# AVianEco/Softspoken

Measured on AMD Instinct MI355X. Metric: audio-seconds processed/sec (whole node), 16 kHz mono, higher is better.
Workload: dtype f16x2

## Files before the change

softspoken_amd/csrc/conv4.hip:

```cpp
#include "conv4_forms.h"
#include <cstdio>
#include <cstdlib>
#include <type_traits>
#include <utility>

namespace ss {

static constexpr int kMfmaPrio = 2;
__device__ __forceinline__ uint32_t relu_pk(uint32_t v) {
    return __builtin_bit_cast(uint32_t, __builtin_elementwise_max(__builtin_bit_cast(s16x2, v), s16x2{0, 0}));
}
__device__ __forceinline__ uint32_t max_pk(uint32_t a, uint32_t b) {
    return __builtin_bit_cast(uint32_t, __builtin_elementwise_max(__builtin_bit_cast(s16x2, a), __builtin_bit_cast(s16x2, b)));
}

template <int NT, int NW, bool BRES, bool RES, bool RADD, bool POOL, int RP, bool FIRST, bool FLAT, bool PF2, bool SPLIT = false, bool RANK1 = false,
          int NH = 1, bool GRES = false>
__global__ __launch_bounds__(64 * NW * NH) __attribute__((amdgpu_waves_per_eu((NT <= 2 && !(SPLIT && RES && !BRES && NW == 4 && NH == 1)) ? 4 : 2)))
void conv3x3_v4_kernel(ConvArgs a, int total_tiles, int lds_b_bytes) {
    constexpr int KC = 32;
    constexpr bool DUO = NH > 1;
    static_assert(!DUO || (NT == 1 && NW * NH == 16 && (RP == 0 || (GRES && RP == 1 && POOL)) && !FIRST && !FLAT && !PF2),
                  "DUO: the plain A / B launches; GRES also conv2_1.B's projection in B");
    static_assert(!GRES || (DUO && BRES && SPLIT && !RES), "GRES: f16x2 B launches with resident banks");
    constexpr bool RING = DUO && !BRES;
    static_assert(!RING || (SPLIT && NH == 4), "RING: f16x2, four 4-wave tiles");
    static_assert(!SPLIT || !PF2, "SPLIT: single-stage prefetch");
    static_assert(!RANK1 || (SPLIT && !RES && !RADD), "RANK1: conv1_1.B in f16x2 mode");
    static_assert(!(FIRST && SPLIT) || RANK1, "FIRST in f16x2 mode: the block's residual is the fp32 rank-1 term");
    static_assert(!FLAT || (NT == 1 && NW == 8 && BRES && (RADD || RP) && !POOL && !FIRST), "FLAT: conv9_1.B");
    static_assert(!PF2 || (BRES && !FIRST), "two-stage prefetch: resident-weight launches");
    static_assert(RP == 0 || (!RES && !RADD && !FIRST), "RP: a B launch that computes the block's projection itself (no r tensor)");
    static_assert(!FIRST || (NT == 1 && BRES && !RES && !RADD), "FIRST: conv1_1.B, one 32 -> 32 chunk, rank-1 residual");
    constexpr int kTapBytes = 2 * NT * 1024;
    constexpr int TAPS = RES ? 10 : 9;
    constexpr int NTHR = 64 * NW;
    constexpr int TH = 2 * NW;
    constexpr int PR = TH + 2;
    constexpr int kA = PR * kRowPitch;
    constexpr int NPA = PR * kPatch * 4;
    constexpr int AIT = (NPA + NTHR - 1) / NTHR;
    constexpr int NPB = (SPLIT ? 2 : 1) * TAPS * kTapBytes / 16;
    constexpr int BIT = BRES ? 1 : (DUO ? (NPB / 2 + NTHR - 1) / NTHR : (NPB + NTHR - 1) / NTHR);
    static_assert(!(RES && (RADD || POOL)), "RES is the A launch; RADD / POOL belong to B launches");
    static_assert(AIT <= 4, "edge flags are packed 8 bits per piece");
    extern __shared__ __attribute__((aligned(16))) char smem[];

    const int half = DUO ? __builtin_amdgcn_readfirstlane((int)threadIdx.x / NTHR) : 0;
    const int tid = DUO ? (int)threadIdx.x % NTHR : (int)threadIdx.x, lane = tid & 63;
    const int wave = __builtin_amdgcn_readfirstlane(tid >> 6);
    const int hh = lane >> 5, m = lane & 31;
    const int py = (m >> 1) & 1, px = (m & 1) | ((m >> 2) << 1);
    char* sA = smem + half * kA;
    const int sb_bytes = RING ? 2 * lds_b_bytes : lds_b_bytes;
    char* sB = smem + NH * kA;
    const int proj_steps = RP ? (a.C0x + a.C1x) / 16 : 0;
    constexpr bool proj_lds = RP > 0 && (BRES || NT == 3 || SPLIT);
    const char* sProj = smem + NH * kA + sb_bytes;
    const int proj_tiles = SPLIT ? a.Cout / 32 : NT;
    const int proj_bank = proj_steps * proj_tiles * 1024;
    const float* sBias = (const float*)(sProj + (proj_lds ? (SPLIT ? 2 : 1) * proj_bank : 0));
    constexpr int FW = 20, FROWS = PR + 3;
    float* sFb = (float*)sBias + 32;
    float* sF = sFb + 32;
    float* sFlat = (float*)sBias + 32;

    const int H = a.H, W = a.W, Cout = a.Cout;
    const int ngroups = Cout / (32 * NT);
    const int nch_r = (a.C0 + a.C1) / KC;
    const int nch = SPLIT ? 2 * nch_r : nch_r;
    const int all_taps = nch_r * TAPS;

    const int xcd = blockIdx.x & 7, local = (int)(blockIdx.x >> 3) * NH + half, gper = (int)(gridDim.x >> 3) * NH;
    const int per = (total_tiles + 7) >> 3;
#ifdef SS_DEVBUILD
// ... 424 lines not shown
                const int tiles = Cout / 32;
#pragma unroll
                for (int k = 0; k < RP; ++k) {
                    const int sidx = ci * RP + k < proj_steps ? ci * RP + k : 0;
#pragma unroll
                    for (int nt = 0; nt < NT; ++nt)
                        wpg[k][nt] = *(const u32x4*)((const char*)a.proj_w + ((size_t)(sidx * tiles + cur.g * NT + nt) * 64 + lane) * 16);
                }
            }
        }
        if (ci == 0) {
#pragma unroll
            for (int nt = 0; nt < NT; ++nt)
#pragma unroll
                for (int g = 0; g < 4; ++g) {
                    const f32x4 b4 = *(const f32x4*)(sBias + co0 + nt * 32 + 8 * g + 4 * hh);
                    acc[nt][4 * g] = b4[0]; acc[nt][4 * g + 1] = b4[1]; acc[nt][4 * g + 2] = b4[2]; acc[nt][4 * g + 3] = b4[3];
                    if constexpr (RES) {
                        const f32x4 r4 = *(const f32x4*)(sBias + Cout + co0 + nt * 32 + 8 * g + 4 * hh);
                        racc[nt][4 * g] = r4[0]; racc[nt][4 * g + 1] = r4[1]; racc[nt][4 * g + 2] = r4[2]; racc[nt][4 * g + 3] = r4[3];
                    }
                }
        }
        auto proj_products = [&](auto k0c, auto k1c) {
            constexpr int K0 = decltype(k0c)::value, K1 = decltype(k1c)::value;
#pragma unroll
            for (int k = K0; k < K1; ++k) {
                const int sidx = (ci >> 1) * RP + k < proj_steps ? (ci >> 1) * RP + k : 0;
#pragma unroll
                for (int nt = 0; nt < NT; ++nt) {
                    const int wt = (sidx * proj_tiles + (int)(co0 >> 5) + nt) * 1024 + lane * 16;
                    const u32x4 wh = *(const u32x4*)(sProj + wt), wl = *(const u32x4*)(sProj + proj_bank + wt);
                    acc[nt] = mfma16<true>(wh, pxl[k - K0], acc[nt]);
                    acc[nt] = mfma16<true>(wl, pxh[k - K0], acc[nt]);
                    acc[nt] = mfma16<true>(wh, pxh[k - K0], acc[nt]);
                }
            }
        };
        using KZ_ = std::integral_constant<int, 0>; using KH_ = std::integral_constant<int, RPH>; using KR_ = std::integral_constant<int, RP>;
        if constexpr (SPLIT && RP > 0 && PART == 1) {
            proj_products(KZ_{}, KH_{});
            __builtin_amdgcn_sched_barrier(0);
            if constexpr (RP > RPH) issue_proj(cur, ci >> 1, KH_{}, KR_{});
        }
        if constexpr (FLAT && SPLIT && RP > 0) load_flat_w();
        {
            const char* bbase = sB + boff0 + (BRES ? ((DUO && !GRES ? cur.g * nch : 0) + (SPLIT ? (ci >> 1) * 2 : ci)) * TAPS * kTapBytes
                                                   : RING ? ((stage_no >> 1) & 1) * lds_b_bytes : 0);
            constexpr int PD = (NT == 1) ? 4 : 2;
            u32x4 af[PD], bfr[PD][NT];
            u32x4 rfr[RES ? 2 : 1][RES ? NT : 1];
            if (a.dbg & 32) __builtin_amdgcn_s_setprio(kMfmaPrio);
            constexpr bool kMerged = SPLIT && NSTEP == 36 && NT == 1;
            if constexpr (kMerged) {
                constexpr int PM = 3;
                u32x4 pf[PM], wh_[PM], wl_[PM], rh_[RES ? 2 : 1], rl_[RES ? 2 : 1];
                const char* bb0 = bbase; const char* bb1 = bbase + TAPS * kTapBytes;
                auto load3 = [&](int st, int slot) {
                    const int tap = st >> 1, sub = st & 1, dy = tap / 3, dx = tap % 3;
                    pf[slot] = *(const u32x4*)(sA + aoff0 + dy * kRowPitch + dx * kPixPitch + sub * 32);
                    wh_[slot] = *(const u32x4*)(bb0 + tap * kTapBytes + sub * 1024);
                    wl_[slot] = *(const u32x4*)(bb1 + tap * kTapBytes + sub * 1024);
                };
#pragma unroll
                for (int st = 0; st < PM - 1; ++st) load3(st, st);
#pragma unroll
                for (int st = 0; st < 18; ++st) {
                    if (st + PM - 1 < 18) load3(st + PM - 1, (st + PM - 1) % PM);
                    if constexpr (RES) {
                        if (st == 6) {
#pragma unroll
                            for (int sub = 0; sub < 2; ++sub) {
                                rh_[sub] = *(const u32x4*)(bb0 + 9 * kTapBytes + sub * 1024);
                                rl_[sub] = *(const u32x4*)(bb1 + 9 * kTapBytes + sub * 1024);
                            }
                        }
                    }
                    const u32x4 pixv = pf[st % PM];
                    acc[0] = mfma16<true>(wh_[st % PM], pixv, acc[0]);
                    acc[0] = mfma16<true>(wl_[st % PM], pixv, acc[0]);
                    if constexpr (RES) {
                        if (st == 8 || st == 9) {
                            racc[0] = mfma16<true>(rh_[st & 1], pixv, racc[0]);
                            racc[0] = mfma16<true>(rl_[st & 1], pixv, racc[0]);
                        }
                    }
                }
            } else
#pragma unroll
            for (int bank = 0; bank < NSTEP / 18; ++bank) {
                const char* bb = bbase + bank * TAPS * kTapBytes;
                auto load_frags = [&](int st, u32x4& fa, u32x4 (&fbb)[NT]) {
                    const int tap = st >> 1, sub = st & 1, dy = tap / 3, dx = tap % 3;
                    fa = *(const u32x4*)(sA + aoff0 + dy * kRowPitch + dx * kPixPitch + sub * 32);
#pragma unroll
                    for (int nt = 0; nt < NT; ++nt) fbb[nt] = *(const u32x4*)(bb + tap * kTapBytes + (sub * NT + nt) * 1024);
                };
                if (bank) __builtin_amdgcn_sched_barrier(0);
#pragma unroll
                for (int st = 0; st < PD - 1; ++st) load_frags(st, af[st], bfr[st]);
#pragma unroll
                for (int st = 0; st < 18; ++st) {
                    if (st + PD - 1 < 18) load_frags(st + PD - 1, af[(st + PD - 1) % PD], bfr[(st + PD - 1) % PD]);
                    if constexpr (RES) {
                        if (st == 6) {
#pragma unroll
                            for (int sub = 0; sub < 2; ++sub)
#pragma unroll
                                for (int nt = 0; nt < NT; ++nt) rfr[sub][nt] = *(const u32x4*)(bb + 9 * kTapBytes + (sub * NT + nt) * 1024);
                        }
                    }
                    const u32x4 pixv = af[st % PD];
#pragma unroll
                    for (int nt = 0; nt < NT; ++nt) {
                        acc[nt] = mfma16<SPLIT>(bfr[st % PD][nt], pixv, acc[nt]);
                        if constexpr (RES) {
                            if (st == 8 || st == 9) racc[nt] = mfma16<SPLIT>(rfr[st & 1][nt], pixv, racc[nt]);
                        }
                    }
                }
            }
        }

        if constexpr (SPLIT && RP > RPH && PART == 1) proj_products(KH_{}, KR_{});
        if constexpr (RP > 0 && !SPLIT) {
#pragma unroll
            for (int k = 0; k < RP; ++k) {
                const int sidx = ci * RP + k < proj_steps ? ci * RP + k : 0;
#pragma unroll
                for (int nt = 0; nt < NT; ++nt) {
                    u32x4 wp;
                    if constexpr (proj_lds) wp = *(const u32x4*)(sProj + (sidx * NT + nt) * 1024 + lane * 16); else wp = wpg[k][nt];
                    acc[nt] = __builtin_amdgcn_mfma_f32_32x32x16_bf16(__builtin_bit_cast(bf16x8, wp), __builtin_bit_cast(bf16x8, xf[k]), acc[nt], 0, 0, 0);
                }
            }
        }
        if (a.dbg & 32) __builtin_amdgcn_s_setprio(0);
        if constexpr (FIRST && !SPLIT) {
            const float f = sF[(2 * wave + py + 2) * FW + px + 2];
// ... 294 lines not shown
            return false;
        }
        cs = n1; n1 = n2; ok1 = ok2;
        if constexpr (PF2) { n2 = n3; ok2 = ok3; }
        return true;
    };
    using P0 = std::integral_constant<int, 0>; using P1 = std::integral_constant<int, 1>;
    if constexpr (DUO) {
        for (int i = 0; i < half; ++i) lds_barrier();
        for (int s = 0; s < max_stages; s += SPLIT ? 2 : 1) {
            if (s < my_stages) {
                stage(P0{}, ra0);
                if constexpr (SPLIT) stage(P1{}, ra0);
            } else {
                lds_barrier(); ring_duty(s, max_stages >> 1); lds_barrier();
                if constexpr (SPLIT) { lds_barrier(); ring_duty(s + 1, max_stages >> 1); lds_barrier(); }
            }
        }
        for (int i = half; i < NH - 1; ++i) lds_barrier();
    } else if constexpr (SPLIT) {
        while (stage(P0{}, ra0) && stage(P1{}, ra0)) {}
    } else if constexpr (PF2) {
        while (stage(P0{}, ra0) && stage(P0{}, ra1)) {}
    } else {
        while (stage(P0{}, ra0)) {}
    }
#ifdef SS_DEVBUILD
    if (a.stamps && lane == 0) {
        uint32_t* p = (uint32_t*)a.stamps + (((size_t)blockIdx.x * NH + half) * NW + wave) * 16;
        for (int i = 0; i < 5; ++i) p[i] = st_sum[i];
        p[5] = (uint32_t)jit_n; p[6] = st_sum[5]; p[7] = st_sum[6]; p[8] = st_sum[7]; p[9] = st_sum[8]; p[10] = st_sum[9]; p[11] = st_sum[10]; p[12] = st_sum[11];
    }
#endif
}

template <int NT, int NW, bool BRES, bool RES, bool RADD, bool POOL, int RP, bool FIRST, bool FLAT, bool PF2, bool SPLIT = false, bool RANK1 = false,
          int NH = 1, bool GRES = false>
static hipError_t launch_v4_k(const ConvArgs& a, int total, int lds_b, size_t lds, int grid, hipStream_t s) {
    static std::atomic<uint64_t> attr_done{0};
    if (hipError_t e = allow_full_lds((const void*)conv3x3_v4_kernel<NT, NW, BRES, RES, RADD, POOL, RP, FIRST, FLAT, PF2, SPLIT, RANK1, NH, GRES>, attr_done)) return e;
    hipLaunchKernelGGL((conv3x3_v4_kernel<NT, NW, BRES, RES, RADD, POOL, RP, FIRST, FLAT, PF2, SPLIT, RANK1, NH, GRES>), dim3(grid), dim3(64 * NW * NH),
                       lds, s, a, total, lds_b);
    return hipGetLastError();
}

typedef hipError_t (*V4Launch)(const ConvArgs&, int, int, size_t, int, hipStream_t);
#define SS_V4_LAUNCH(...) &launch_v4_k<__VA_ARGS__>,
static const V4Launch kV4Launch[] = {SS_V4_FORMS(SS_V4_LAUNCH)};
#undef SS_V4_LAUNCH
static_assert(sizeof kV4Launch / sizeof kV4Launch[0] == kV4FormCount, "one launch function per form");

int conv_v4_flat_groups() { return 128 / 16; }

bool conv_v4_supports(const ConvArgs& a_in, int NT, int num_cus, int prec) {
    ConvArgs a = a_in;
    return choose_v4(a, NT, num_cus, prec).ok;
}

const char* conv_v4_variant(const ConvArgs& a_in, int NT, int num_cus, int prec) {
    ConvArgs a = a_in;
    const V4Choice c = choose_v4(a, NT, num_cus, prec);
    return c.ok ? v4_form_name(c.form) : "conv3x3_v4_kernel<invalid>";
}

hipError_t launch_conv3x3_v4(const ConvArgs& a_in, int NT, int num_cus, int prec, hipStream_t s) {
    ConvArgs a = a_in;
    const V4Choice c = choose_v4(a, NT, num_cus, prec);
    const int i = c.ok ? v4_form_index(c.form) : -1;
    if (i < 0) return hipErrorInvalidValue;
    return kV4Launch[i](a, c.total, c.lds_b, c.lds, c.grid, s);
}

}
```

softspoken_amd/csrc/conv4_forms.h:

```cpp
#pragma once
#include "kernels.h"
#include "mfma_util.h"
#include <algorithm>
#include <cstdio>

namespace ss {

static constexpr int kPixPitch = 80;
static constexpr int kRowPitch = 1664;
static constexpr int kPatch = 18;

struct V4Form { int NT, NW; bool BRES, RES, RADD, POOL; int RP; bool FIRST, FLAT, PF2, SPLIT, RANK1; int NH; bool GRES; };
constexpr bool operator==(const V4Form& a, const V4Form& b) {
    return a.NT == b.NT && a.NW == b.NW && a.BRES == b.BRES && a.RES == b.RES && a.RADD == b.RADD && a.POOL == b.POOL && a.RP == b.RP &&
           a.FIRST == b.FIRST && a.FLAT == b.FLAT && a.PF2 == b.PF2 && a.SPLIT == b.SPLIT && a.RANK1 == b.RANK1 && a.NH == b.NH && a.GRES == b.GRES;
}

#define SS_V4_FORMS(X)                                                                                                                \
                                                                                               \
    X(1, 4, 0, 0, 0, 0, 0, 0, 0, 0, 0, 0, 1, 0) X(1, 4, 0, 0, 1, 0, 0, 0, 0, 0, 0, 0, 1, 0) X(1, 4, 0, 0, 1, 1, 0, 0, 0, 0, 0, 0, 1, 0)  \
    X(1, 4, 0, 1, 0, 0, 0, 0, 0, 0, 0, 0, 1, 0) X(1, 4, 1, 0, 0, 0, 0, 0, 0, 0, 0, 0, 1, 0) X(1, 4, 1, 0, 1, 0, 0, 0, 0, 0, 0, 0, 1, 0)  \
    X(1, 4, 1, 0, 1, 1, 0, 0, 0, 0, 0, 0, 1, 0) X(1, 4, 1, 1, 0, 0, 0, 0, 0, 0, 0, 0, 1, 0)                                              \
    X(2, 4, 0, 0, 0, 0, 0, 0, 0, 0, 0, 0, 1, 0) X(2, 4, 0, 0, 1, 0, 0, 0, 0, 0, 0, 0, 1, 0) X(2, 4, 0, 0, 1, 1, 0, 0, 0, 0, 0, 0, 1, 0)  \
    X(2, 4, 0, 1, 0, 0, 0, 0, 0, 0, 0, 0, 1, 0) X(2, 4, 1, 0, 0, 0, 0, 0, 0, 0, 0, 0, 1, 0) X(2, 4, 1, 0, 1, 0, 0, 0, 0, 0, 0, 0, 1, 0)  \
// ... 137 lines not shown
        const int nh = 4, thd = 32 / nh;
        const V4Form f = form_of(16 / nh, true, nh, true);
        const size_t group_b = (size_t)all_taps * tap_bytes * banks;
        const size_t proj_b = proj ? (size_t)((a.C0x + a.C1x) / 16) * (a.Cout / 32) * 1024 * banks : 0;
        const size_t lds = nh * (size_t)(thd + 2) * kRowPitch + group_b + proj_b + (size_t)a.Cout * 4;
        const long total_pos = (long)a.N * (a.H / thd) * a.tiles_x;
        const int grid = total_pos <= 0x7fffffff / ngroups ? gres_grid(num_cus, (int)total_pos, ngroups, nh) : 0;
        if (v4_form_index(f) >= 0 && lds <= 160 * 1024 && gres_grid_ok(grid, ngroups)) {
            c.lds_b = (int)group_b;
            a.tiles_y = a.H / thd;
            c.total = (int)(total_pos * ngroups);
            return accept(f, grid, lds);
        }
    }
    if ((duo_env == 2 || duo_env == 4) && split && (nw == 8 || (duo_env == 4 && duo8_env))) {
        const int nh = duo_env, thd = 32 / nh;
        const size_t fixed = nh * (size_t)(thd + 2) * kRowPitch + (size_t)a.Cout * 4 * (a.res_out ? 2 : 1);
        const size_t chunk_b = (size_t)taps * tap_bytes * banks;
        const size_t all_b = (size_t)ngroups * all_taps * tap_bytes * banks;
        const bool bres_d = fixed + all_b <= 160 * 1024;
        static const int ring_env = dev_env("SOFTSPOKEN_RING", 1);
        const bool ring = !bres_d && nh == 4 && ring_env && (a.res_out != nullptr || ring_env == 2 || (a.H <= 32 && a.res_in != nullptr));
        const size_t lds = fixed + (bres_d ? all_b : 2 * chunk_b);
        const V4Form f = form_of(16 / nh, bres_d, nh, false);
        if ((bres_d || ring) && v4_form_index(f) >= 0 && lds <= 160 * 1024) {
            c.lds_b = (int)(bres_d ? all_b : chunk_b);
            a.tiles_y = a.H / thd;
            c.total = (int)((long)a.N * a.tiles_y * a.tiles_x * ngroups);
            int grid = (num_cus + 7) / 8 * 8;
            if (grid * nh > c.total) grid = ((c.total + nh - 1) / nh + 7) / 8 * 8;
            return accept(f, grid, lds);
        }
    }
    const size_t lds = (size_t)(th + 2) * kRowPitch + c.lds_b + (size_t)a.Cout * 4 * (a.res_out ? 2 : 1) + (first ? (size_t)(32 + (th + 5) * 20) * 4 : 0) +
                       (flat ? (size_t)nw * 2 * 64 * 4 : 0) + (proj && (ngroups == 1 || split) ? (size_t)((a.C0x + a.C1x) / 16) * (split ? a.Cout / 32 : NT) * 1024 * banks : 0);
    V4Form f = form_of(nw, bres, 1, false);
    static const int pf2_env = dev_env("SOFTSPOKEN_PF2", 1);
    if (pf2_env && bres && !first && !flat && NT <= 2 && lds * 3 > 160 * 1024) {
        V4Form p = f;
        p.PF2 = true;
        if (v4_form_index(p) >= 0) f = p;
    }
    if (v4_form_index(f) < 0) return c;
    int bpc = (int)((160 * 1024) / lds);
    if (bpc < 1) return c;
    if (bpc > 3) bpc = 3;
    { static const int cap = dev_env("SOFTSPOKEN_BPC", 3); if (bpc > cap) bpc = cap; }
    int grid = num_cus * bpc;
    if (grid > c.total) grid = c.total;
    grid = (grid + 7) / 8 * 8;
    return accept(f, grid, lds);
}

}
```

softspoken_amd/csrc/engine.h:

```cpp
#pragma once
#include "../../include/softspoken.h"
#include "kernels.h"

#include <map>
#include <set>
#include <string>
#include <vector>

namespace ss {

inline size_t pcm_bytes_per_sample(int format) {
    switch (format) {
        case SS_PCM_U8: case SS_PCM_S8: return 1;
        case SS_PCM_S16: case SS_PCM_S16BE: return 2;
        case SS_PCM_S24: case SS_PCM_S24BE: return 3;
        case SS_PCM_F64: case SS_PCM_F64BE: return 8;
        default: return 4;
    }
}

int fail(ss_ctx* c, int code, const std::string& msg);
const char* thread_error();

#define HIPCHK(c, expr)                                                                                   \
    do {                                                                                                  \
        hipError_t e_ = (expr);                                                                           \
        if (e_ != hipSuccess)                                                                             \
            return ss::fail((c), SS_ERR_HIP, std::string(#expr) + ": " + hipGetErrorString(e_));          \
    } while (0)

struct BlobEntry { char name[96]; uint32_t dtype, ndim; int64_t shape[4]; uint64_t offset, nbytes; };
static_assert(sizeof(BlobEntry) == 152, "blob entry layout");
struct Blob {
    std::map<std::string, BlobEntry> e;
    const char* base = nullptr;
    size_t size = 0;
    bool has(const std::string& k) const { return e.count(k) != 0; }
    const float* f32(const std::string& k, size_t count, std::string& err) const;
};
bool parse_blob(const void* p, size_t n, Blob& b, std::string& err);

enum Precision { kFp32 = 0, kBf16 = 1, kF16x2 = 2 };

struct ConvPlan {
    std::string name;
    void* d_w2 = nullptr; float* d_bias2 = nullptr; float* d_res_bias = nullptr; float* d_rank1 = nullptr;
    void* d_w3 = nullptr; void* d_proj = nullptr; float* d_bias3 = nullptr;
    void* d_w_ups = nullptr;
    bool s1_range_proven = false;
    void* d_w_s1 = nullptr;
    void* d_w_s16 = nullptr;
    void* d_w_upsr = nullptr;
    void* d_w_ups32 = nullptr;
    int ups32_nt = 1;
    int Cout = 0, NT = 1, C0 = 0, C1 = 0, R0 = 0, R1 = 0, H = 0, W = 0;
};

struct FileRec {
    int64_t off = 0;
    int64_t n = 0;
    int64_t n_padded = 0;
    double duration = 0;
    int64_t W = 0, win_base = 0;
    int64_t bin_off = 0; int n_bins = 0;
};

struct StreamSet;
struct SepState;

struct SepPlan {
    int N = 0, hop = 0;
    int64_t W = 0, n_bins = 0, windows_run = 0;
    std::vector<ss_separation_range> ranges;
};

struct Workspace {
    int chunk = 0; int64_t bytes = 0;
    std::map<std::string, void*> act;
    void* arena = nullptr;
    int64_t lo_delta = 0;
    float* feat = nullptr; float* flat = nullptr;
    int flat_groups = 0;
};

struct RunMerger {
    double brk = 0; bool have = false; ss_region cur{0, 0}; int64_t reg0 = 0, reg1 = 0;
    void add(int64_t first_bin, int64_t last_bin, std::vector<ss_region>& out, std::vector<int64_t>* bins = nullptr);
    void flush(std::vector<ss_region>& out, std::vector<int64_t>* bins = nullptr);
};

struct KStat { std::string name; int64_t launches = 0; double ms = 0, flops = 0, bytes = 0, issued = 0; };
struct PendingEvt { int sid; hipEvent_t a, b; };

}

struct ss_ctx {
    int device = 0;
    uint32_t flags = 0;
    ss::Precision prec = ss::kFp32;
    bool bf16 = false;
// ... 138 lines not shown
```

softspoken_amd/csrc/engine.hip:

```cpp
#include "engine.h"

#include <algorithm>
#include <chrono>
#include <cmath>
#include <cstdio>
#include <cstdlib>
#include <cstring>

namespace ss {

static thread_local std::string g_err;

int fail(ss_ctx* c, int code, const std::string& msg) {
    g_err = msg;
    if (c) c->err = msg;
    return code;
}
const char* thread_error() { return g_err.c_str(); }

double now_ms() { return std::chrono::duration<double, std::milli>(std::chrono::steady_clock::now().time_since_epoch()).count(); }

static int stat_id(ss_ctx* c, const std::string& name) {
    for (size_t i = 0; i < c->stats.size(); ++i) if (c->stats[i].name == name) return (int)i;
    KStat k; k.name = name; c->stats.push_back(k);
// ... 210 lines not shown
        const int nt = p.ups32_nt, mtw = dev_env("SOFTSPOKEN_UPS32_MTW", 2) == 2 && nt < 3 ? 2 : 1;
        if (conv_ups32_supports(au, nt, mtw, cus))
            return go(conv_ups32_variant(nt, mtw), au, issued_ups, [&](ConvArgs& x) { return launch_conv3x3_ups32(x, nt, mtw, cus, stream); });
    }
    if (c->prec == kF16x2 && ex.first_w && p.d_w_s16 && dev_env("SOFTSPOKEN_C1S", 1)) {
        ConvArgs as = a;
        const int form = dev_env("SOFTSPOKEN_C1S_FORM", 16) == 32 && p.d_w_s1 ? 32 : 16;
        as.wpk = form == 16 ? p.d_w_s16 : p.d_w_s1;
        as.relu = 1 | (dev_env("SOFTSPOKEN_C1S_ABLATE", 0) << 4);
        as.plain = p.s1_range_proven && dev_env("SOFTSPOKEN_C1S_TRACK", 0) == 0;
        if (conv1_stream_supports(as)) {
            const int rows = dev_env("SOFTSPOKEN_C1S_ROWS", 32);
            if (int rc = go(conv1_stream_variant(as, form), as, -1.0, [&](ConvArgs& x) { return launch_conv1_stream(x, form, rows, cus, stream); })) return rc;
            if (dev_env("SOFTSPOKEN_C1S", 1) != 2) return SS_OK;
        }
    }
    if (c->prec != kFp32 && dev_env("SOFTSPOKEN_CONV4", 1) && conv_v4_supports(a, p.NT, cus, prec4)) {
        if (int rc = go(conv_v4_variant(a, p.NT, cus, prec4), a, -1.0, [&](ConvArgs& x) { return launch_conv3x3_v4(x, p.NT, cus, prec4, stream); })) return rc;
        if (ex.flat_part) ws.flat_groups = conv_v4_flat_groups();
        return SS_OK;
    }
    if (c->prec == kF16x2) return fail(c, SS_ERR_STATE, "f16x2: no kernel form for " + p.name);
    if (ex.flat_part) ws.flat_groups = conv_v2_flat_groups(c->bf16);
    return go(conv_v2_variant(a, c->bf16, p.NT, cus), a, -1.0, [&](ConvArgs& x) { return launch_conv3x3_v2(x, c->bf16, p.NT, cus, stream); });
}

static int run_block_proj(ss_ctx* c, Workspace& ws, hipStream_t stream, const ConvPlan& pa, const ConvPlan& pb, int n, const void* x0, const void* x1,
                          void* h, void* out, void* pool, const ConvExtra& ex = ConvExtra()) {
    if ((c->prec != kBf16 && c->prec != kF16x2) || !pa.d_w3 || !pb.d_proj) return 1;
    const int prec4 = c->prec == kF16x2 ? 2 : 1;
    const int cus = c->num_cus;
    const double es = c->prec == kBf16 ? 2 : 4;
    ConvArgs a{}, b{};
    a.lo_delta = b.lo_delta = ws.lo_delta; a.range_flag = b.range_flag = c->d_range_flag;
    a.src0 = x0; a.src1 = x1; a.wpk = pa.d_w3; a.bias = pa.d_bias2; a.out = h; a.plain = 1;
    a.N = n; a.H = pa.H; a.W = pa.W; a.Cout = pa.Cout; a.C0 = pa.C0; a.C1 = pa.C1; a.relu = 1;
    b.src0 = h; b.wpk = pb.d_w2; b.bias = pb.d_bias3; b.out = out; b.pool_out = pool;
    b.N = n; b.H = pb.H; b.W = pb.W; b.Cout = pb.Cout; b.C0 = pb.Cout; b.C1 = 0; b.relu = 1;
    b.proj_w = pb.d_proj; b.xp0 = x0; b.xp1 = x1; b.C0x = pa.C0; b.C1x = pa.C1;
    b.flat_w4 = ex.flat_w4; b.flat_part = ex.flat_part; b.store_out = ex.store_out;
    a.dbg = b.dbg = base_dbg();
    ConvArgs au = a;
    au.wpk = pa.d_w_ups;
    const bool ups = c->prec == kF16x2 && pa.d_w_ups && x1 && conv_ups_supports(au, cus);
    if ((!ups && !conv_v4_supports(a, pa.NT, cus, prec4)) || !conv_v4_supports(b, pb.NT, cus, prec4)) return 1;
    mark_written(c, ws, h); mark_written(c, ws, pool);
    if (ex.store_out) mark_written(c, ws, out);
    const double px = (double)n * pa.H * pa.W, cin = pa.C0 + pa.C1, cinb = pa.C0 + pa.C1 / 4.0;
    const double flops_a = 2.0 * px * pa.Cout * 9.0 * cin, bytes_a = px * es * (cinb + pa.Cout);
    auto v4 = [&](const ConvPlan& p, ConvArgs& x, double flops, double bytes) {
        return conv_launch(c, stream, conv_v4_variant(x, p.NT, cus, prec4), p.name, x, flops, bytes, -1.0,
                           [&](ConvArgs& y) { return launch_conv3x3_v4(y, p.NT, cus, prec4, stream); });
    };
    int rc;
    if (ups) {
        ScopedLaunch sl(c, stream, std::string(conv_ups_variant()) + "/" + pa.name, flops_a, bytes_a, px * pa.Cout * (9.0 * pa.C0 + 4.0 * pa.C1));
        HIPCHK(c, launch_conv3x3_ups(au, cus, stream));
    } else if ((rc = v4(pa, a, flops_a, bytes_a))) return rc;
    const double flops_b = 2.0 * px * pb.Cout * (9.0 * pb.Cout + cin) + (ex.flat_part ? 2.0 * px * 32 * 4 : 0.0);
    const double bytes_b = px * es * (pb.Cout + cinb + (ex.flat_part && !ex.store_out ? 0 : pb.Cout) + (pool ? pb.Cout / 4.0 : 0));
    if ((rc = v4(pb, b, flops_b, bytes_b))) return rc;
    if (ex.flat_part) ws.flat_groups = conv_v4_flat_groups();
    return SS_OK;
}

static int forward_chunk_(ss_ctx* c, Workspace& ws, hipStream_t stream, const float* signal, const int64_t* d_winoff, int n, float* d_logits, float* d_spec);

int forward_chunk(ss_ctx* c, Workspace& ws, hipStream_t stream, const float* signal, const int64_t* d_winoff, int n, float* d_logits, float* d_spec) {
#ifdef SS_DEVBUILD
    c->dbg_written.clear(); c->dbg_n = n; c->dbg_ws = (int)(&ws - c->ws);
    c->dbg_written.insert("feat");
    if (d_logits) c->dbg_written.insert("flat_part");
    const int rc = forward_chunk_(c, ws, stream, signal, d_winoff, n, d_logits, d_spec);
    if (rc) { c->dbg_written.clear(); c->dbg_n = 0; }
    return rc;
#else
    return forward_chunk_(c, ws, stream, signal, d_winoff, n, d_logits, d_spec);
#endif
}

static int forward_chunk_(ss_ctx* c, Workspace& ws, hipStream_t stream, const float* signal, const int64_t* d_winoff, int n, float* d_logits, float* d_spec) {
    FrontendTables tb{c->d_pretw, c->d_w2048, c->d_mel_start, c->d_mel_count, c->d_mel_off, c->d_mel_w, c->mel_nw, c->d_mel_wp, dev_env("SOFTSPOKEN_FEDBG", 0),
                      c->d_win2, c->d_twt, c->d_wkt, c->d_mel_wq, c->d_mel_p0};
    float* const feat = ws.feat;
    {
        ScopedLaunch sl(c, stream, "frontend", 0.0, (double)n * (66150.0 * 4 + 128.0 * 256 * 4));
        HIPCHK(c, launch_frontend(signal, d_winoff, n, tb, feat, c->num_cus, stream));
    }
    if (!d_logits) return SS_OK;
    auto A = [&](const char* k) -> void* {
        auto it = ws.act.find(k);
        return it == ws.act.end() ? nullptr : it->second;
    };
    const double es = c->prec == kBf16 ? 2 : 4;
    const std::vector<ConvPlan>& cv = c->convs;
    int rc, i = 0;
#define RC2(x) if ((rc = (x))) return rc
    {
        ConvExtra ex; ex.first_w = c->d_first_w; ex.first_b = c->d_first_b;
        RC2(run_conv2(c, ws, stream, cv[i++], n, nullptr, nullptr, A("c1"), A("p1"), nullptr, nullptr, feat, ex));
    }
    struct Blk { const char *x0, *x1, *h, *r, *y, *pool; };
    const Blk blks[] = {{"p1", nullptr, "h2", "r2", "c2", "p2"},   {"p2", nullptr, "h3", "r3", "c3", "p3"},
                        {"p3", nullptr, "h4", "r4", "c4", "p4"},   {"p4", nullptr, "hb", "rb", "bott", nullptr},
                        {"bott", nullptr, "he", "re", "enc", nullptr}, {"c4", "enc", "h6", "r6", "c6", nullptr},
                        {"c3", "c6", "h7", "r7", "c7", nullptr},   {"c2", "c7", "h8", "r8", "c8", nullptr}};
    const bool proj = c->prec != kFp32 && dev_env("SOFTSPOKEN_CONV4", 1) && dev_env("SOFTSPOKEN_RPROJ", 1);
    for (const Blk& b : blks) {
// ... 348 lines not shown
```

softspoken_amd/csrc/kernels.h:

```cpp
#pragma once
#include <hip/hip_runtime.h>
#include <stdint.h>
#include <atomic>
#include <cstdlib>

namespace ss {

#ifdef SS_DEVBUILD
static inline int dev_env(const char* name, int dflt) { const char* v = getenv(name); return v ? atoi(v) : dflt; }
#else
static constexpr int dev_env(const char*, int dflt) { return dflt; }
#endif

inline hipError_t allow_full_lds(const void* kernel, std::atomic<uint64_t>& done) {
    int dev = 0;
    hipError_t e = hipGetDevice(&dev);
    if (e != hipSuccess) return e;
    const uint64_t bit = 1ull << (dev & 63);
    if (done.load(std::memory_order_acquire) & bit) return hipSuccess;
    e = hipFuncSetAttribute(kernel, hipFuncAttributeMaxDynamicSharedMemorySize, 160 * 1024);
    if (e == hipSuccess) done.fetch_or(bit, std::memory_order_release);
    return e;
}

// ... 25 lines not shown
    void* stamps;
};
static constexpr bool kOrderSideBySide = true;
struct RingItem { int pos, g; };
__host__ __device__ inline int ring_lim(int xcd, int total_pos) {
    const int per_pos = (total_pos + 7) >> 3, left = total_pos - xcd * per_pos;
    return left < 0 ? 0 : left < per_pos ? left : per_pos;
}
__host__ __device__ inline int ring_group0(int wg, int ngroups, bool seq) { return seq ? 0 : wg % ngroups; }
__host__ __device__ inline int ring_group_step(int G, int ngroups, bool seq) { return seq ? 1 % ngroups : G % ngroups; }
__host__ __device__ inline RingItem ring_item(int xcd, int wg, int G, int item, int tile, int total_pos, int ngroups, bool seq) {
    const int lim = ring_lim(xcd, total_pos);
    int quad, g;
    if (seq) { quad = wg + (item / ngroups) * G; g = item % ngroups; }
    else { const int j = wg + item * G; quad = j / ngroups; g = j - quad * ngroups; }
    const int idx = 4 * quad + tile;
    return RingItem{idx < lim ? xcd * ((total_pos + 7) >> 3) + idx : -1, g};
}
__host__ __device__ inline int ring_items(int xcd, int wg, int G, int tile, int total_pos, int ngroups, bool seq) {
    const int lim = ring_lim(xcd, total_pos);
    const int quads = lim > tile ? (lim - tile + 3) >> 2 : 0;
    if (seq) return quads > wg ? (quads - wg + G - 1) / G * ngroups : 0;
    const int n = quads * ngroups;
    return n > wg ? (n - wg + G - 1) / G : 0;
}

__host__ __device__ inline bool gres_grid_ok(int grid, int ngroups) { return grid > 0 && ngroups > 0 && grid % (8 * ngroups) == 0; }
__host__ __device__ inline int gres_grid(int num_cus, int total_pos, int ngroups, int nh) {
    int G = (num_cus + 7) / 8;
    if (ngroups <= 0 || G % ngroups) return 0;
    const int units = (((total_pos + 7) >> 3) + nh - 1) / nh;
    if (units < G / ngroups) G = (units > 0 ? units : 1) * ngroups;
    return 8 * G;
}
__host__ __device__ inline int gres_group(int wg, int ngroups) { return wg % ngroups; }
__host__ __device__ inline RingItem gres_item(int xcd, int wg, int G, int item, int tile, int total_pos, int ngroups, int nh) {
    const int lim = ring_lim(xcd, total_pos), S = G / ngroups;
    const int idx = (wg / ngroups + item * S) * nh + tile;
    return RingItem{idx < lim ? xcd * ((total_pos + 7) >> 3) + idx : -1, wg % ngroups};
}
__host__ __device__ inline int gres_items(int xcd, int wg, int G, int tile, int total_pos, int ngroups, int nh) {
    const int lim = ring_lim(xcd, total_pos), S = G / ngroups, s = wg / ngroups;
    const int units = lim > tile ? (lim - tile + nh - 1) / nh : 0;
    return units > s ? (units - s + S - 1) / S : 0;
}

hipError_t launch_conv3x3_v2(const ConvArgs& a, bool bf16, int NT, int num_cus, hipStream_t s);
const char* conv_v2_variant(const ConvArgs& a, bool bf16, int NT, int num_cus);
int conv_v2_flat_groups(bool bf16);
bool conv_v4_supports(const ConvArgs& a, int NT, int num_cus, int prec);
const char* conv_v4_variant(const ConvArgs& a, int NT, int num_cus, int prec);
int conv_v4_flat_groups();
hipError_t launch_conv3x3_v4(const ConvArgs& a, int NT, int num_cus, int prec, hipStream_t s);

bool conv_ups_supports(const ConvArgs& a, int num_cus);
const char* conv_ups_variant();
size_t conv_ups_weight_bytes(int C0, int C1);
hipError_t launch_conv3x3_ups(const ConvArgs& a, int num_cus, hipStream_t s);
bool conv_upsr_supports(const ConvArgs& a, int num_cus);
const char* conv_upsr_variant();
size_t conv_upsr_weight_bytes(int C0, int C1, int Cout);
hipError_t launch_conv3x3_upsr(const ConvArgs& a, int num_cus, hipStream_t s);

bool conv_ups32_supports(const ConvArgs& a, int NT, int MTW, int num_cus);
const char* conv_ups32_variant(int NT, int MTW);
size_t conv_ups32_weight_bytes(int C0, int C1, int Cout);
hipError_t launch_conv3x3_ups32(const ConvArgs& a, int NT, int MTW, int num_cus, hipStream_t s);

bool conv1_stream_supports(const ConvArgs& a);
const char* conv1_stream_variant(const ConvArgs& a, int form);
size_t conv1_stream_weight_bytes();
hipError_t launch_conv1_stream(const ConvArgs& a, int form, int rows_per_unit, int num_cus, hipStream_t s);

struct Head1dWeights { float w1[4][4][3], b1[4], w2[4][4][3], wr[4][4], b2r[4], wo[4], bo, fscale; };
hipError_t launch_mask_head_parts(const float* parts, int n_parts, const float* flat_bias, const Head1dWeights& hw, float* logits,
                                  int N, hipStream_t s);
hipError_t launch_spec_tail(const void* x, int64_t lo_delta, const float* w , const float* bias, float* spec, int N, int prec,
                            hipStream_t s);

static constexpr int kMelLo = 10, kMelHi = 32, kMelPitch = 43;
struct FrontendTables {
    const float4* pretw;
    const float2* w2048;
    const int* mel_start;
    const int* mel_count;
    const int* mel_off;
    const float* mel_w;
    int mel_nw;
    const float* mel_wp;
    int dbg;
    const float2* win2;
    const float2* twt;
    const float2* wkt;
    const float* mel_wq;
    const int* mel_p0;
};
static constexpr int kMelPairsLo = 9, kMelPairsHi = 20, kMelRow = 60;
static constexpr int kPwWords = 816;
hipError_t launch_frontend(const float* arena, const int64_t* win_off, int n, const FrontendTables& t, float* feat,
                           int num_cus, hipStream_t s);

struct BatchFile { int64_t pcm_off; int64_t frames; int64_t mono_off; int64_t out_off; int64_t n_out; };
hipError_t launch_decode_mono_batch(const void* pcm, int format, int channels, const BatchFile* d_files, int n_files,
                                    int64_t max_frames, float* mono, hipStream_t s);
hipError_t launch_stft512_mag(const float* x, int64_t n, int64_t n_frames, float* out, int num_cus, hipStream_t s);
hipError_t launch_silence_encode(const void* pcm, int format, int channels, int64_t frames, const int64_t* d_ranges, int n_ranges,
// ... 31 lines not shown
```

softspoken_amd/csrc/weights.hip:

```cpp
#include "engine.h"

#include <algorithm>
#include <cmath>
#include <cstring>

namespace ss {

const float* Blob::f32(const std::string& k, size_t count, std::string& err) const {
    auto it = e.find(k);
    if (it == e.end()) { err = "weights blob: missing tensor '" + k + "'"; return nullptr; }
    if (it->second.dtype != 0 || it->second.nbytes != count * 4) {
        err = "weights blob: tensor '" + k + "' has wrong dtype/size"; return nullptr;
    }
    return (const float*)(base + it->second.offset);
}

bool parse_blob(const void* p, size_t n, Blob& b, std::string& err) {
    if (n < 16 || memcmp(p, "SSWBLOB1", 8) != 0) { err = "weights blob: bad magic"; return false; }
    uint32_t cnt; memcpy(&cnt, (const char*)p + 8, 4);
    if (16 + (size_t)cnt * sizeof(BlobEntry) > n) { err = "weights blob: truncated table"; return false; }
    b.base = (const char*)p; b.size = n;
    for (uint32_t i = 0; i < cnt; ++i) {
        BlobEntry en; memcpy(&en, (const char*)p + 16 + (size_t)i * sizeof(BlobEntry), sizeof(BlobEntry));
        en.name[95] = 0;
// ... 458 lines not shown
            if (pk.size() != conv1_stream_weight_bytes()) return fail(c, SS_ERR_STATE, "pack_conv_stream16: size");
            if ((rc = dev_upload(c, (char**)&B.d_w_s16, pk.data(), pk.size()))) return rc;
#ifdef SS_DEVBUILD
            pack_conv_stream(f2, pk, c->split_range_ok);
            if ((rc = dev_upload(c, (char**)&B.d_w_s1, pk.data(), pk.size()))) return rc;
#endif
            const double fmax = 6.2076;
            std::vector<double> bh(cout);
            double worst = 0;
            for (int co = 0; co < cout; ++co) {
                double q = std::fabs((double)f1.b[co]);
                for (int t = 0; t < 9; ++t) q += std::fabs((double)f1.w[(size_t)co * 9 + t]) * fmax;
                bh[co] = q; worst = std::max(worst, q);
            }
            for (int co = 0; co < cout; ++co) {
                double q = std::fabs((double)b2r[co]) + std::fabs((double)fr.w[co]) * fmax;
                for (int ci = 0; ci < cout; ++ci)
                    for (int t = 0; t < 9; ++t) q += std::fabs((double)f2.w[((size_t)co * cout + ci) * 9 + t]) * bh[ci];
                worst = std::max(worst, q);
            }
            B.s1_range_proven = std::isfinite(worst) && worst < 60000.0;
        }
        c->convs.push_back(B);
        return SS_OK;
    }
    const int NTA = (c->prec == kF16x2 && NT == 3) ? 1 : NT;
    ConvPlan A; A.name = name + ".A"; A.Cout = cout; A.NT = NTA; A.C0 = cin0; A.C1 = cin1; A.H = H; A.W = W;
    if ((rc = dev_upload(c, &A.d_bias2, f1.b.data(), cout * 4))) return rc;
    if (c->prec == kF16x2) pack_conv_split(f1, &fr, NTA, pk, c->split_range_ok); else pack_conv_v2(f1, &fr, c->bf16, NT, pk);
    if ((rc = dev_upload(c, (char**)&A.d_w2, pk.data(), pk.size()))) return rc;
    if ((rc = dev_upload(c, &A.d_res_bias, fr.b.data(), cout * 4))) return rc;
    if (c->prec == kF16x2 && NTA == 1 && cin0 >= 64 && cin0 % 32 == 0 && cin1 % 32 == 0 && (cin1 >= 32 || dev_env("SOFTSPOKEN_UPSR", 1) >= 2)) {
        pack_conv_split_upsr(f1, fr, cin0, cin1, pk, c->split_range_ok);
        if (pk.size() != conv_upsr_weight_bytes(cin0, cin1, cout)) return fail(c, SS_ERR_STATE, "pack_conv_split_upsr: size");
        if ((rc = dev_upload(c, (char**)&A.d_w_upsr, pk.data(), pk.size()))) return rc;
    }
    if (c->prec == kFp32 && cin1 >= 16 && cin0 % 16 == 0 && cin1 % 16 == 0 && cout % 32 == 0 && H % 16 == 0 && dev_env("SOFTSPOKEN_UPS32", 1)) {
        A.ups32_nt = dev_env("SOFTSPOKEN_UPS32_NT", 1);
        if (A.ups32_nt < 1 || A.ups32_nt > 3 || (cout / 32) % A.ups32_nt) A.ups32_nt = 1;
        pack_conv_v2_ups(f1, fr, cin0, cin1, A.ups32_nt, pk);
        if (pk.size() != conv_ups32_weight_bytes(cin0, cin1, cout)) return fail(c, SS_ERR_STATE, "pack_conv_v2_ups: size");
        if ((rc = dev_upload(c, (char**)&A.d_w_ups32, pk.data(), pk.size()))) return rc;
    }
    c->convs.push_back(A);
    if (c->bf16) {
        pack_conv_v2(f1, nullptr, true, NT, pk);
        if ((rc = dev_upload(c, (char**)&A.d_w3, pk.data(), pk.size()))) return rc;
        c->convs.back().d_w3 = A.d_w3;
    }
    if (c->prec == kF16x2) {
        pack_conv_split(f1, nullptr, NTA, pk, c->split_range_ok);
        if ((rc = dev_upload(c, (char**)&A.d_w3, pk.data(), pk.size()))) return rc;
        c->convs.back().d_w3 = A.d_w3;
        if (cin1 >= 32 && cin0 >= 32 && cout == 32) {
            pack_conv_split_ups(f1, cin0, cin1, pk, c->split_range_ok);
            if (pk.size() != conv_ups_weight_bytes(cin0, cin1)) return fail(c, SS_ERR_STATE, "pack_conv_split_ups: size");
            if ((rc = dev_upload(c, (char**)&A.d_w_ups, pk.data(), pk.size()))) return rc;
            c->convs.back().d_w_ups = A.d_w_ups;
        }
    }
    const int NTB = (c->prec == kF16x2 && NT == 3 && dev_env("SOFTSPOKEN_NTB1", 1)) ? 1 : NT;
    ConvPlan B; B.name = name + ".B"; B.Cout = cout; B.NT = NTB; B.C0 = cout; B.R0 = cin0; B.R1 = cin1; B.H = H; B.W = W;
    if (c->bf16 && cin % 16 == 0) {
        const int steps = cin / 16, tiles = cout / 32;
        std::vector<uint16_t> pj((size_t)steps * tiles * 64 * 8);
        for (int st = 0; st < steps; ++st) for (int t = 0; t < tiles; ++t) for (int l = 0; l < 64; ++l) for (int j = 0; j < 8; ++j)
            pj[(((size_t)st * tiles + t) * 64 + l) * 8 + j] = f2bf(fr.w[(size_t)(32 * t + (l & 31)) * cin + 16 * st + 8 * (l >> 5) + j]);
        if ((rc = dev_upload(c, (char**)&B.d_proj, (const char*)pj.data(), pj.size() * 2))) return rc;
        if ((rc = dev_upload(c, &B.d_bias3, b2r.data(), cout * 4))) return rc;
    }
    if (c->prec == kF16x2 && cin % 16 == 0) {
        const int steps = cin / 16, tiles = cout / 32;
        const size_t bank = (size_t)steps * tiles * 64 * 8;
        std::vector<uint16_t> pj(2 * bank);
        for (int st = 0; st < steps; ++st) for (int t = 0; t < tiles; ++t) for (int l = 0; l < 64; ++l) for (int j = 0; j < 8; ++j) {
            const float v = fr.w[(size_t)(32 * t + (l & 31)) * cin + 16 * st + 8 * (l >> 5) + j];
            const uint16_t hi = f2h(v);
            if ((hi & 0x7c00u) == 0x7c00u) c->split_range_ok = false;
            const size_t at = (((size_t)st * tiles + t) * 64 + l) * 8 + j;
            pj[at] = hi; pj[bank + at] = f2h(v - h2f(hi));
        }
        if ((rc = dev_upload(c, (char**)&B.d_proj, (const char*)pj.data(), pj.size() * 2))) return rc;
        if ((rc = dev_upload(c, &B.d_bias3, b2r.data(), cout * 4))) return rc;
    }
    if (c->prec == kF16x2) pack_conv_split(f2, nullptr, NTB, pk, c->split_range_ok); else pack_conv_v2(f2, nullptr, c->bf16, NT, pk);
    if ((rc = dev_upload(c, (char**)&B.d_w2, pk.data(), pk.size()))) return rc;
    if ((rc = dev_upload(c, &B.d_bias2, f2.b.data(), cout * 4))) return rc;
    c->convs.push_back(B);
    return SS_OK;
}

int build_model(ss_ctx* c, const Blob& bl) {
    int rc;
    c->split_range_ok = true;
    struct RB { const char* n; int c0, c1, co, H, W; const char *x0, *x1, *h, *y, *pool; };
    const RB rbs[] = {{"conv1_1", 1, 0, 32, 128, 256, nullptr, nullptr, "h1", "c1", "p1"},
                      {"conv2_1", 32, 0, 64, 64, 128, "conv1_1", nullptr, "h2", "c2", "p2"},
                      {"conv3_1", 64, 0, 96, 32, 64, "conv2_1", nullptr, "h3", "c3", "p3"},
                      {"conv4_1", 96, 0, 128, 16, 32, "conv3_1", nullptr, "h4", "c4", "p4"},
                      {"conv_bottleneck", 128, 0, 128, 8, 16, "conv4_1", nullptr, "hb", "bott", nullptr},
                      {"encoder_out", 128, 0, 128, 8, 16, "conv_bottleneck", nullptr, "he", "enc", nullptr},
                      {"conv6", 128, 128, 96, 16, 32, "conv4_1", "encoder_out", "h6", "c6", nullptr},
                      {"conv7", 96, 96, 64, 32, 64, "conv3_1", "conv6", "h7", "c7", nullptr},
                      {"conv8", 64, 64, 32, 64, 128, "conv2_1", "conv7", "h8", "c8", nullptr},
                      {"conv9_1", 32, 32, 32, 128, 256, "conv1_1", "conv8", "h9", "c9", nullptr},
                      {"spec_output_conv.0", 32, 0, 32, 128, 256, "conv9_1", nullptr, "hs", "s9", nullptr}};
// ... 105 lines not shown
```

Before: 31200.

## Add wide NT=2 f16x2 conv A path for 64-channel outputs

Adds a wide variant of the f16x2 DUO conv kernel in which each wave computes two 32-channel output tiles (NT=2). Each pixel fragment loaded from LDS is reused across both tiles, and the per-tap merged loop uses a 3-deep prefetch. The variant is selected by default for plain Cout=64 A convolutions that the narrow NT=1 form would otherwise handle, and a separately packed NT=2 weight buffer is uploaded for it. It is meant to halve activation-fragment LDS traffic and tile launches per output channel. In exchange it uses more registers and more LDS for resident weight banks, and it duplicates weight memory.

```diff
diff --git a/softspoken_amd/csrc/conv4.hip b/softspoken_amd/csrc/conv4.hip
--- a/softspoken_amd/csrc/conv4.hip
+++ b/softspoken_amd/csrc/conv4.hip
@@ -20,7 +20,8 @@
 void conv3x3_v4_kernel(ConvArgs a, int total_tiles, int lds_b_bytes) {
     constexpr int KC = 32;
     constexpr bool DUO = NH > 1;
-    static_assert(!DUO || (NT == 1 && NW * NH == 16 && (RP == 0 || (GRES && RP == 1 && POOL)) && !FIRST && !FLAT && !PF2),
+    static_assert(!DUO || ((NT == 1 || (NT == 2 && BRES && !RES && !RADD && RP == 0 && SPLIT)) && NW * NH == 16 &&
+                           (RP == 0 || (GRES && RP == 1 && POOL)) && !FIRST && !FLAT && !PF2),
                   "DUO: the plain A / B launches; GRES also conv2_1.B's projection in B");
     static_assert(!GRES || (DUO && BRES && SPLIT && !RES), "GRES: f16x2 B launches with resident banks");
     constexpr bool RING = DUO && !BRES;
@@ -551,6 +552,7 @@
             u32x4 rfr[RES ? 2 : 1][RES ? NT : 1];
             if (a.dbg & 32) __builtin_amdgcn_s_setprio(kMfmaPrio);
             constexpr bool kMerged = SPLIT && NSTEP == 36 && NT == 1;
+            constexpr bool kMerged2 = SPLIT && NSTEP == 36 && NT == 2;
             if constexpr (kMerged) {
                 constexpr int PM = 3;
                 u32x4 pf[PM], wh_[PM], wl_[PM], rh_[RES ? 2 : 1], rl_[RES ? 2 : 1];
@@ -584,6 +586,30 @@
                             racc[0] = mfma16<true>(rl_[st & 1], pixv, racc[0]);
                         }
                     }
+                }
+            } else if constexpr (kMerged2) {
+                constexpr int PM2 = 3;
+                u32x4 pf[PM2], wh_[PM2][NT], wl_[PM2][NT];
+                const char* bb0 = bbase; const char* bb1 = bbase + TAPS * kTapBytes;
+                auto load5 = [&](int st, int slot) {
+                    const int tap = st >> 1, sub = st & 1, dy = tap / 3, dx = tap % 3;
+                    pf[slot] = *(const u32x4*)(sA + aoff0 + dy * kRowPitch + dx * kPixPitch + sub * 32);
+#pragma unroll
+                    for (int nt = 0; nt < NT; ++nt) {
+                        wh_[slot][nt] = *(const u32x4*)(bb0 + tap * kTapBytes + (sub * NT + nt) * 1024);
+                        wl_[slot][nt] = *(const u32x4*)(bb1 + tap * kTapBytes + (sub * NT + nt) * 1024);
+                    }
+                };
+#pragma unroll
+                for (int st = 0; st < PM2 - 1; ++st) load5(st, st);
+#pragma unroll
+                for (int st = 0; st < 18; ++st) {
+                    if (st + PM2 - 1 < 18) load5(st + PM2 - 1, (st + PM2 - 1) % PM2);
+                    const u32x4 pixv = pf[st % PM2];
+#pragma unroll
+                    for (int nt = 0; nt < NT; ++nt) acc[nt] = mfma16<true>(wh_[st % PM2][nt], pixv, acc[nt]);
+#pragma unroll
+                    for (int nt = 0; nt < NT; ++nt) acc[nt] = mfma16<true>(wl_[st % PM2][nt], pixv, acc[nt]);
                 }
             } else
 #pragma unroll
@@ -984,6 +1010,26 @@
 
 int conv_v4_flat_groups() { return 128 / 16; }
 
+static constexpr V4Launch kV4WideLaunch = &launch_v4_k<2, 4, true, false, false, false, 0, false, false, false, true, false, 4, false>;
+
+bool conv_v4_wide_supports(const ConvArgs& a_in, int num_cus, int prec) {
+    ConvArgs a = a_in;
+    return choose_v4_wide(a, num_cus, prec).ok;
+}
+
+const char* conv_v4_wide_variant(const ConvArgs& a_in, int num_cus, int prec) {
+    ConvArgs a = a_in;
+    const V4Choice c = choose_v4_wide(a, num_cus, prec);
+    return c.ok ? v4_form_name(c.form) : "conv3x3_v4_kernel<invalid>";
+}
+
+hipError_t launch_conv3x3_v4_wide(const ConvArgs& a_in, int num_cus, int prec, hipStream_t s) {
+    ConvArgs a = a_in;
+    const V4Choice c = choose_v4_wide(a, num_cus, prec);
+    if (!c.ok || !(c.form == kV4WideForm)) return hipErrorInvalidValue;
+    return kV4WideLaunch(a, c.total, c.lds_b, c.lds, c.grid, s);
+}
+
 bool conv_v4_supports(const ConvArgs& a_in, int NT, int num_cus, int prec) {
     ConvArgs a = a_in;
     return choose_v4(a, NT, num_cus, prec).ok;
diff --git a/softspoken_amd/csrc/conv4_forms.h b/softspoken_amd/csrc/conv4_forms.h
--- a/softspoken_amd/csrc/conv4_forms.h
+++ b/softspoken_amd/csrc/conv4_forms.h
@@ -213,4 +213,31 @@
     return accept(f, grid, lds);
 }
 
-}
+#ifndef SS_WIDE_DEFAULT
+#define SS_WIDE_DEFAULT 1
+#endif
+static constexpr V4Form kV4WideForm{2, 4, true, false, false, false, 0, false, false, false, true, false, 4, false};
+static constexpr V4Form kV4WideFrom{1, 4, true, false, false, false, 0, false, false, false, true, false, 4, false};
+
+inline V4Choice choose_v4_wide(ConvArgs& a, int num_cus, int prec) {
+    V4Choice c{};
+    static const int wide_env = dev_env("SOFTSPOKEN_WIDE", SS_WIDE_DEFAULT);
+    static const int rproj_env = dev_env("SOFTSPOKEN_RPROJ", SS_RPROJ_DEFAULT);
+    if (!wide_env || !rproj_env || prec != 2 || !a.plain || a.Cout != 64) return c;
+    ConvArgs narrow = a;
+    const V4Choice n = choose_v4(narrow, 1, num_cus, prec);
+    if (!n.ok || !(n.form == kV4WideFrom)) return c;
+    const int nh = 4, thd = 32 / nh;
+    const size_t banks_b = (size_t)((a.C0 + a.C1) / 32) * 9 * (2 * 2 * 1024) * 2;
+    const size_t lds = nh * (size_t)(thd + 2) * kRowPitch + banks_b + (size_t)a.Cout * 4;
+    if (lds > 160 * 1024) return c;
+    a.tiles_y = a.H / thd; a.tiles_x = a.W / 16;
+    c.total = (int)((long)a.N * a.tiles_y * a.tiles_x);
+    c.lds_b = (int)banks_b;
+    int grid = (num_cus + 7) / 8 * 8;
+    if (grid * nh > c.total) grid = ((c.total + nh - 1) / nh + 7) / 8 * 8;
+    c.form = kV4WideForm; c.grid = grid; c.block = 64 * kV4WideForm.NW * kV4WideForm.NH; c.lds = lds; c.ok = true;
+    return c;
+}
+
+}
diff --git a/softspoken_amd/csrc/engine.h b/softspoken_amd/csrc/engine.h
--- a/softspoken_amd/csrc/engine.h
+++ b/softspoken_amd/csrc/engine.h
@@ -46,6 +46,7 @@
     std::string name;
     void* d_w2 = nullptr; float* d_bias2 = nullptr; float* d_res_bias = nullptr; float* d_rank1 = nullptr;
     void* d_w3 = nullptr; void* d_proj = nullptr; float* d_bias3 = nullptr;
+    void* d_w3_wide = nullptr;
     void* d_w_ups = nullptr;
     bool s1_range_proven = false;
     void* d_w_s1 = nullptr;
diff --git a/softspoken_amd/csrc/engine.hip b/softspoken_amd/csrc/engine.hip
--- a/softspoken_amd/csrc/engine.hip
+++ b/softspoken_amd/csrc/engine.hip
@@ -286,8 +286,14 @@
         return conv_launch(c, stream, conv_v4_variant(x, p.NT, cus, prec4), p.name, x, flops, bytes, -1.0,
                            [&](ConvArgs& y) { return launch_conv3x3_v4(y, p.NT, cus, prec4, stream); });
     };
+    ConvArgs aw = a;
+    aw.wpk = pa.d_w3_wide;
+    const bool wide = !ups && c->prec == kF16x2 && pa.d_w3_wide && conv_v4_wide_supports(aw, cus, prec4);
     int rc;
-    if (ups) {
+    if (wide) {
+        if ((rc = conv_launch(c, stream, conv_v4_wide_variant(aw, cus, prec4), pa.name, aw, flops_a, bytes_a, -1.0,
+                              [&](ConvArgs& y) { return launch_conv3x3_v4_wide(y, cus, prec4, stream); }))) return rc;
+    } else if (ups) {
         ScopedLaunch sl(c, stream, std::string(conv_ups_variant()) + "/" + pa.name, flops_a, bytes_a, px * pa.Cout * (9.0 * pa.C0 + 4.0 * pa.C1));
         HIPCHK(c, launch_conv3x3_ups(au, cus, stream));
     } else if ((rc = v4(pa, a, flops_a, bytes_a))) return rc;
diff --git a/softspoken_amd/csrc/kernels.h b/softspoken_amd/csrc/kernels.h
--- a/softspoken_amd/csrc/kernels.h
+++ b/softspoken_amd/csrc/kernels.h
@@ -101,6 +101,9 @@
 const char* conv_v4_variant(const ConvArgs& a, int NT, int num_cus, int prec);
 int conv_v4_flat_groups();
 hipError_t launch_conv3x3_v4(const ConvArgs& a, int NT, int num_cus, int prec, hipStream_t s);
+bool conv_v4_wide_supports(const ConvArgs& a, int num_cus, int prec);
+const char* conv_v4_wide_variant(const ConvArgs& a, int num_cus, int prec);
+hipError_t launch_conv3x3_v4_wide(const ConvArgs& a, int num_cus, int prec, hipStream_t s);
 
 bool conv_ups_supports(const ConvArgs& a, int num_cus);
 const char* conv_ups_variant();
diff --git a/softspoken_amd/csrc/weights.hip b/softspoken_amd/csrc/weights.hip
--- a/softspoken_amd/csrc/weights.hip
+++ b/softspoken_amd/csrc/weights.hip
@@ -534,6 +534,11 @@
         pack_conv_split(f1, nullptr, NTA, pk, c->split_range_ok);
         if ((rc = dev_upload(c, (char**)&A.d_w3, pk.data(), pk.size()))) return rc;
         c->convs.back().d_w3 = A.d_w3;
+        if (NTA == 1 && cout == 64 && cin % 32 == 0 && (size_t)(cin / 32) * 9 * 4096 * 2 <= (size_t)72 * 1024) {
+            pack_conv_split(f1, nullptr, 2, pk, c->split_range_ok);
+            if ((rc = dev_upload(c, (char**)&A.d_w3_wide, pk.data(), pk.size()))) return rc;
+            c->convs.back().d_w3_wide = A.d_w3_wide;
+        }
         if (cin1 >= 32 && cin0 >= 32 && cout == 32) {
             pack_conv_split_ups(f1, cin0, cin1, pk, c->split_range_ok);
             if (pk.size() != conv_ups_weight_bytes(cin0, cin1)) return fail(c, SS_ERR_STATE, "pack_conv_split_ups: size");
```

New measurement: 31440, median of 6. Within noise of the previous version (+0.7%).
